# linto-ai/whisper-timestamped

Measured on NVIDIA H100. Metric: audio-sec/s (RTF) large-v3 1h synthetic @1/2/4/8 H100; DTW GB/s vs HBM peak, higher is better.
Workload: dtype bf16x3 tensor-core GEMMs (float32-accurate), f32 elsewhere, f64 DTW accumulate

## Files before the change

### whisper-timestamped_b200/csrc/gemm_tc.cu

```cuda
#include <cuda_bf16.h>

#include <stdlib.h>

#include "sm90.cuh"

namespace wts {

constexpr int BM = 128, BN = 128, BK = 64;
constexpr int TILE_BYTES = BM * BK * 2;
constexpr int STAGES = 3;
constexpr int STAGE_BYTES = 4 * TILE_BYTES;
constexpr int GT_THREADS = 288;
constexpr int PT_THREADS = 384;
constexpr int PT_PRODUCER_REGS = 40, PT_CONSUMER_REGS = 232;
static_assert(128 * PT_PRODUCER_REGS + 256 * PT_CONSUMER_REGS <= 65536, "setmaxnreg plan exceeds the register file");
constexpr int GROUP_M = 8;
constexpr int GT_SMEM = STAGES * STAGE_BYTES + 256 + 1024;
constexpr int PART_LD = BN + 4;
static_assert(BM * PART_LD * 4 <= STAGES * STAGE_BYTES, "the partial tile lives in the operand ring");

__device__ __forceinline__ float gelu_erf_tc(float v) { return 0.5f * v * (1.0f + erff(v * 0.70710678118654752440f)); }

struct TcArgs {
    WtsGemm g;
    int a_has_bo, a_has_bi, b_has_bo, b_has_bi;
    int split_k;
    int pair_stores;
};

__device__ __forceinline__ int64_t out_offset(const WtsGemm& g, int m, int n, int64_t ld)
{
    return g.head_dim > 0 ? (int64_t)(n / g.head_dim) * g.head_stride + (int64_t)m * ld + (n % g.head_dim)
                          : (int64_t)m * ld + n;
}

__device__ __forceinline__ void store_one(const WtsGemm& g, int m, int n, float t, float* of, __nv_bfloat16* ob)
{
    if (of) of[out_offset(g, m, n, g.ldc)] = t;
    if (ob) {
        const __nv_bfloat16 hi = __float2bfloat16_rn(t);
        __nv_bfloat16* d = ob + out_offset(g, m, n, g.ldo);
        d[0] = hi;
        d[g.o_plane] = __float2bfloat16_rn(t - __bfloat162float(hi));
    }
}

__device__ __forceinline__ float2 pair_values(const WtsGemm& g, int n, bool two, float v0, float v1, float bias_m, const float* res)
{
    float t0 = g.alpha * v0, t1 = g.alpha * v1;
    if (g.bias) {
        t0 += g.bias_on_m ? bias_m : g.bias[n];
        if (two) t1 += g.bias_on_m ? bias_m : g.bias[n + 1];
    }
    if (g.act == 1) { t0 = gelu_erf_tc(t0); t1 = gelu_erf_tc(t1); }
    if (res) { t0 += res[n]; if (two) t1 += res[n + 1]; }
    return make_float2(t0, t1);
}

__device__ __forceinline__ void store_pair_sb16(__nv_bfloat16* dh, int64_t plane, float t0, float t1)
{
    const __nv_bfloat162 hi = __floats2bfloat162_rn(t0, t1);
    const __nv_bfloat162 lo = __floats2bfloat162_rn(t0 - __low2float(hi), t1 - __high2float(hi));
    *reinterpret_cast<__nv_bfloat162*>(dh) = hi;
    *reinterpret_cast<__nv_bfloat162*>(dh + plane) = lo;
}

__device__ __forceinline__ void epilogue_pair(const WtsGemm& g, int m, int n, float v0, float v1, float bias_m,
                                              const float* res, float* of, __nv_bfloat16* ob)
{
    const bool two = n + 1 < g.N;
    const float2 t = pair_values(g, n, two, v0, v1, bias_m, res);
    const float t0 = t.x, t1 = t.y;
    const bool same_head = g.head_dim == 0 || (n % g.head_dim) + 1 < g.head_dim;
    if (!(two && same_head)) {
        store_one(g, m, n, t0, of, ob);
        if (two) store_one(g, m, n + 1, t1, of, ob);
        return;
    }
    if (of) {
        float* d = of + out_offset(g, m, n, g.ldc);
        if ((reinterpret_cast<uintptr_t>(d) & 7) == 0) *reinterpret_cast<float2*>(d) = make_float2(t0, t1);
        else { d[0] = t0; d[1] = t1; }
    }
    if (ob) {
        __nv_bfloat16* dh = ob + out_offset(g, m, n, g.ldo);
        __nv_bfloat16* dl = dh + g.o_plane;
        if (((reinterpret_cast<uintptr_t>(dh) | reinterpret_cast<uintptr_t>(dl)) & 3) == 0) {
            store_pair_sb16(dh, g.o_plane, t0, t1);
        } else {
            const __nv_bfloat162 hi = __floats2bfloat162_rn(t0, t1);
            const __nv_bfloat162 lo = __floats2bfloat162_rn(t0 - __low2float(hi), t1 - __high2float(hi));
            dh[0] = hi.x; dh[1] = hi.y; dl[0] = lo.x; dl[1] = lo.y;
        }
    }
}

template <bool PAIRS>
__device__ __forceinline__ void epilogue_frag64(const WtsGemm& g, int zo, int zi, int m_base, int n0, const float (&acc)[64])
{
    const int lane = threadIdx.x & 31;
    const int cl = 2 * (lane & 3);
    float* of = g.out_f32 ? g.out_f32 + (int64_t)zo * g.c_bo + (int64_t)zi * g.c_bi : nullptr;
    __nv_bfloat16* ob = g.out_sb16 ? reinterpret_cast<__nv_bfloat16*>(g.out_sb16) + (int64_t)zo * g.o_bo + (int64_t)zi * g.o_bi : nullptr;
#pragma unroll
    for (int i = 0; i < 2; ++i) {
        const int m = m_base + (lane >> 2) + 8 * i;
        if (m >= g.M || (g.row_mask && g.row_mask[m] == 0)) continue;
        const float* res = g.residual ? g.residual + (int64_t)zo * g.r_bo + (int64_t)zi * g.r_bi + (int64_t)m * g.ldr : nullptr;
        const float bias_m = (g.bias && g.bias_on_m) ? g.bias[m] : 0.f;
#pragma unroll
        for (int j = 0; j < 16; ++j) {
            const int n = n0 + cl + 8 * j;
            if (PAIRS) {
                const float2 t = pair_values(g, n, true, acc[4 * j + 2 * i], acc[4 * j + 2 * i + 1], bias_m, res);
                if (of) *reinterpret_cast<float2*>(of + out_offset(g, m, n, g.ldc)) = t;
                if (ob) store_pair_sb16(ob + out_offset(g, m, n, g.ldo), g.o_plane, t.x, t.y);
            } else if (n < g.N) {
                epilogue_pair(g, m, n, acc[4 * j + 2 * i], acc[4 * j + 2 * i + 1], bias_m, res, of, ob);
            }
        }
    }
}

__device__ __forceinline__ void named_bar_sync(int id, int n) { asm volatile("bar.sync %0, %1;" ::"r"(id), "r"(n) : "memory"); }
__device__ __forceinline__ void named_bar_arrive(int id, int n) { asm volatile("bar.arrive %0, %1;" ::"r"(id), "r"(n) : "memory"); }

struct TileCoord { int m0, n0, zo, zi; };

__device__ __forceinline__ TileCoord tile_coord(const WtsGemm& g, int t, int tiles_m, int tiles_n)
{
    const int per_batch = tiles_m * tiles_n;
    const int z = t / per_batch;
    int r = t - z * per_batch;
    const int span = GROUP_M * tiles_n;
    const int grp = r / span;
    const int m_first = grp * GROUP_M;
    const int gm = min(GROUP_M, tiles_m - m_first);
    r -= grp * span;
    TileCoord c;
    c.m0 = (m_first + r % gm) * BM;
    c.n0 = (r / gm) * BN;
    c.zo = z / g.batch_inner;
    c.zi = z - c.zo * g.batch_inner;
    return c;
}

__global__ void __launch_bounds__(PT_THREADS, 1)
gemm_tc_kernel(const __grid_constant__ CUtensorMap tmA, const __grid_constant__ CUtensorMap tmB, const TcArgs args)
{
    extern __shared__ unsigned char smem_raw[];
    const WtsGemm& g = args.g;
    const uint32_t base = (smem_addr(smem_raw) + 1023u) & ~1023u;
    const uint32_t bar = base + STAGES * STAGE_BYTES;
    const int wg = threadIdx.x >> 7, warp = (threadIdx.x >> 5) & 3, lane = threadIdx.x & 31;
    const int tiles_n = (g.N + BN - 1) / BN, tiles_m = (g.M + BM - 1) / BM;
    const int tiles = tiles_m * tiles_n * g.batch_outer * g.batch_inner;
    const int nkb = (g.K + BK - 1) / BK;
    pdl_launch();

    if (threadIdx.x == 0) {
        asm volatile("prefetch.tensormap [%0];" ::"l"(&tmA) : "memory");
        asm volatile("prefetch.tensormap [%0];" ::"l"(&tmB) : "memory");
        for (int s = 0; s < STAGES; ++s) { mbar_init(bar + 8 * s, 1); mbar_init(bar + 32 + 8 * s, 4); }
        asm volatile("fence.mbarrier_init.release.cluster;" ::: "memory");
    }
    __syncthreads();
    pdl_wait();

    if (wg == 0) {
        asm volatile("setmaxnreg.dec.sync.aligned.u32 %0;" ::"n"(PT_PRODUCER_REGS));
        if (warp == 0 && lane == 0) {
            int p = 0;
            for (int t = blockIdx.x; t < tiles; t += gridDim.x) {
                const TileCoord tc = tile_coord(g, t, tiles_m, tiles_n);
                const int azo = args.a_has_bo ? tc.zo : 0, azi = args.a_has_bi ? tc.zi : 0;
                const int bzo = args.b_has_bo ? tc.zo : 0, bzi = args.b_has_bi ? tc.zi : 0;
                for (int kb = 0; kb < nkb; ++kb, ++p) {
                    const int s = p % STAGES, u = p / STAGES;
                    mbar_wait(bar + 32 + 8 * s, (u & 1) ^ 1);
                    const uint32_t full = bar + 8 * s;
                    mbar_expect_tx(full, STAGE_BYTES);
                    const uint32_t st = base + s * STAGE_BYTES;
                    const int kc = kb * BK;
                    tma_load_5d(st, &tmA, full, kc, tc.m0, azi, azo, 0);
                    tma_load_5d(st + TILE_BYTES, &tmA, full, kc, tc.m0, azi, azo, 1);
                    tma_load_5d(st + 2 * TILE_BYTES, &tmB, full, kc, tc.n0, bzi, bzo, 0);
                    tma_load_5d(st + 3 * TILE_BYTES, &tmB, full, kc, tc.n0, bzi, bzo, 1);
                }
            }
        }
        return;
    }

    asm volatile("setmaxnreg.inc.sync.aligned.u32 %0;" ::"n"(PT_CONSUMER_REGS));
    const int c = wg - 1;
    float acc[2][64];
    int l = c;
    for (int t = blockIdx.x + c * gridDim.x; t < tiles; t += 2 * gridDim.x, l += 2) {
        if (l > 0) named_bar_sync(1 + c, 256);
#pragma unroll
        for (int h = 0; h < 2; ++h)
#pragma unroll
            for (int i = 0; i < 64; ++i) acc[h][i] = 0.f;
        int p = l * nkb;
        for (int kb = 0; kb < nkb; ++kb, ++p) {
            const int s = p % STAGES;
            mbar_wait(bar + 8 * s, (p / STAGES) & 1);
            const uint32_t st = base + s * STAGE_BYTES;
            const uint64_t a_hi = wg_desc(st), a_lo = wg_desc(st + TILE_BYTES);
            const uint64_t b_hi = wg_desc(st + 2 * TILE_BYTES), b_lo = wg_desc(st + 3 * TILE_BYTES);
            constexpr uint64_t a_half = (TILE_BYTES / 2) >> 4;
            wg_fence();
#pragma unroll
            for (int k = 0; k < BK / 16; ++k) {
                const uint64_t adv = (uint64_t)(k * 2);
#pragma unroll
                for (int h = 0; h < 2; ++h) wgmma_ss_n128(acc[h], a_hi + h * a_half + adv, b_hi + adv, 1);
#pragma unroll
                for (int h = 0; h < 2; ++h) wgmma_ss_n128(acc[h], a_lo + h * a_half + adv, b_hi + adv, 1);
#pragma unroll
                for (int h = 0; h < 2; ++h) wgmma_ss_n128(acc[h], a_hi + h * a_half + adv, b_lo + adv, 1);
            }
            wg_commit();
            wg_wait<1>();
            if (kb > 0 && lane == 0) mbar_arrive(bar + 32 + 8 * ((p - 1) % STAGES));
        }
        if (t + gridDim.x < tiles) named_bar_arrive(2 - c, 256);
        wg_wait<0>();
        if (lane == 0) mbar_arrive(bar + 32 + 8 * ((p - 1) % STAGES));

        const TileCoord tc = tile_coord(g, t, tiles_m, tiles_n);
        const bool pairs = args.pair_stores && tc.n0 + BN <= g.N;
#pragma unroll 1
        for (int h = 0; h < 2; ++h) {
            float v[64];
#pragma unroll
            for (int i = 0; i < 64; ++i) v[i] = h ? acc[1][i] : acc[0][i];
            if (pairs) epilogue_frag64<true>(g, tc.zo, tc.zi, tc.m0 + 64 * h + 16 * warp, tc.n0, v);
            else epilogue_frag64<false>(g, tc.zo, tc.zi, tc.m0 + 64 * h + 16 * warp, tc.n0, v);
        }
    }
}

__global__ void __launch_bounds__(GT_THREADS, 1)
gemm_tc_skinny_kernel(const __grid_constant__ CUtensorMap tmA, const __grid_constant__ CUtensorMap tmB, const TcArgs args)
{
    extern __shared__ unsigned char smem_raw[];
    const WtsGemm& g = args.g;
    const uint32_t base = (smem_addr(smem_raw) + 1023u) & ~1023u;
    const uint32_t bar = base + STAGES * STAGE_BYTES;
    const int warp = threadIdx.x >> 5, lane = threadIdx.x & 31;
    const int n0 = blockIdx.x * BN, m0 = blockIdx.y * BM;
    const int S = args.split_k;
    const int z = S > 1 ? 0 : blockIdx.z, zo = z / g.batch_inner, zi = z - zo * g.batch_inner;
    const int nkb_all = (g.K + BK - 1) / BK;
    const int part_k = S > 1 ? blockIdx.z : 0;
    const int kb0 = (int)((int64_t)part_k * nkb_all / S);
    const int nkb = (int)((int64_t)(part_k + 1) * nkb_all / S) - kb0;
    pdl_launch();

    if (threadIdx.x == 256) {
        asm volatile("prefetch.tensormap [%0];" ::"l"(&tmA) : "memory");
        asm volatile("prefetch.tensormap [%0];" ::"l"(&tmB) : "memory");
        for (int s = 0; s < STAGES; ++s) { mbar_init(bar + 8 * s, 1); mbar_init(bar + 32 + 8 * s, 8); }
        asm volatile("fence.mbarrier_init.release.cluster;" ::: "memory");
    }
    __syncthreads();
    pdl_wait();

    float acc[64];
    if (warp == 8) {
        if (lane == 0) {
            const int azo = args.a_has_bo ? zo : 0, azi = args.a_has_bi ? zi : 0;
            const int bzo = args.b_has_bo ? zo : 0, bzi = args.b_has_bi ? zi : 0;
            for (int kb = 0; kb < nkb; ++kb) {
                const int s = kb % STAGES, u = kb / STAGES;
                mbar_wait(bar + 32 + 8 * s, (u & 1) ^ 1);
                const uint32_t full = bar + 8 * s;
                mbar_expect_tx(full, STAGE_BYTES);
                const uint32_t st = base + s * STAGE_BYTES;
                const int kc = (kb0 + kb) * BK;
                tma_load_5d(st, &tmA, full, kc, m0, azi, azo, 0);
                tma_load_5d(st + TILE_BYTES, &tmA, full, kc, m0, azi, azo, 1);
                tma_load_5d(st + 2 * TILE_BYTES, &tmB, full, kc, n0, bzi, bzo, 0);
                tma_load_5d(st + 3 * TILE_BYTES, &tmB, full, kc, n0, bzi, bzo, 1);
            }
        }
    } else {
        const int wg = warp >> 2;
#pragma unroll
        for (int i = 0; i < 64; ++i) acc[i] = 0.f;
        for (int kb = 0; kb < nkb; ++kb) {
            const int s = kb % STAGES, u = kb / STAGES;
            mbar_wait(bar + 8 * s, u & 1);
            const uint32_t st = base + s * STAGE_BYTES;
            const uint64_t a_hi = wg_desc(st + wg * (TILE_BYTES / 2)), a_lo = wg_desc(st + TILE_BYTES + wg * (TILE_BYTES / 2));
            const uint64_t b_hi = wg_desc(st + 2 * TILE_BYTES), b_lo = wg_desc(st + 3 * TILE_BYTES);
            wg_fence();
#pragma unroll
            for (int k = 0; k < BK / 16; ++k) {
                const uint64_t adv = (uint64_t)(k * 2);
                wgmma_ss_n128(acc, a_hi + adv, b_hi + adv, 1);
                wgmma_ss_n128(acc, a_lo + adv, b_hi + adv, 1);
                wgmma_ss_n128(acc, a_hi + adv, b_lo + adv, 1);
            }
            wg_commit();
            wg_wait<1>();
            if (kb > 0 && lane == 0) mbar_arrive(bar + 32 + 8 * ((kb - 1) % STAGES));
        }
        wg_wait<0>();

        const int rl = 64 * wg + 16 * (warp & 3) + (lane >> 2);
        const int cl = 2 * (lane & 3);
        if (S == 1) {
            epilogue_frag64<false>(g, zo, zi, m0 + 64 * wg + 16 * (warp & 3), n0, acc);
        } else {
            asm volatile("bar.sync 1, 256;" ::: "memory");
            float* part = reinterpret_cast<float*>(smem_raw + (base - smem_addr(smem_raw)));
#pragma unroll
            for (int i = 0; i < 2; ++i)
#pragma unroll
                for (int j = 0; j < 16; ++j)
                    *reinterpret_cast<float2*>(part + (rl + 8 * i) * PART_LD + cl + 8 * j) =
                        make_float2(acc[4 * j + 2 * i], acc[4 * j + 2 * i + 1]);
        }
    }
    if (S > 1) {
        __syncwarp();
        cluster_sync_all();
        if (threadIdx.x < 256) {
            uint32_t rank;
            asm volatile("mov.u32 %0, %%cluster_ctarank;" : "=r"(rank));
            const int c = threadIdx.x & 127, half = threadIdx.x >> 7;
            const int n = n0 + c;
            if (n < g.N) {
                uint32_t peer[8];
#pragma unroll
                for (int s = 0; s < 8; ++s) {
                    peer[s] = 0;
                    if (s < S) asm volatile("mapa.shared::cluster.u32 %0, %1, %2;" : "=r"(peer[s]) : "r"(base + 4u * c), "r"(s));
                }
                const float bias_n = (g.bias && !g.bias_on_m) ? g.bias[n] : 0.f;
                float* of = g.out_f32;
                __nv_bfloat16* ob = reinterpret_cast<__nv_bfloat16*>(g.out_sb16);
#pragma unroll 1
                for (int m = (int)rank + S * half; m < g.M; m += 2 * S) {
                    if (g.row_mask && g.row_mask[m] == 0) continue;
                    float x[8];
#pragma unroll
                    for (int s = 0; s < 8; ++s) {
                        x[s] = 0.f;
                        if (s < S) asm volatile("ld.shared::cluster.f32 %0, [%1];" : "=f"(x[s]) : "r"(peer[s] + (uint32_t)(m * PART_LD * 4)));
                    }
                    float t = 0.f;
#pragma unroll
                    for (int s = 0; s < 8; ++s) t += x[s];
                    t = g.alpha * t + (g.bias ? (g.bias_on_m ? g.bias[m] : bias_n) : 0.f);
                    if (g.act == 1) t = gelu_erf_tc(t);
                    if (g.residual) t += g.residual[(int64_t)m * g.ldr + n];
                    store_one(g, m, n, t, of, ob);
                }
            }
        }
        __syncwarp();
        cluster_sync_all();
    }
}

static int make_map(CUtensorMap* tm, const void* ptr, int64_t K, int64_t rows, int64_t ld, int64_t plane, int64_t n_bi,
                    int64_t s_bi, int64_t n_bo, int64_t s_bo, int box_rows, const char* which)
{
    auto enc = tensor_map_encoder();
    if (!enc) { set_error("wts_gemm: cuTensorMapEncodeTiled entry point not available"); return -4; }
    if ((reinterpret_cast<uintptr_t>(ptr) & 15) || (ld & 7) || (plane & 7) || (s_bi & 7) || (s_bo & 7)) {
        set_error("wts_gemm(tc): operand %s not 16-byte aligned (ptr=%p ld=%lld plane=%lld bi=%lld bo=%lld)", which, ptr,
                  (long long)ld, (long long)plane, (long long)s_bi, (long long)s_bo);
        return -5;
    }
    const int64_t e_bi = s_bi ? n_bi : 1, e_bo = s_bo ? n_bo : 1;
    cuuint64_t dims[5] = {(cuuint64_t)K, (cuuint64_t)rows, (cuuint64_t)e_bi, (cuuint64_t)e_bo, 2};
    const cuuint64_t row_b = (cuuint64_t)ld * 2;
    cuuint64_t strides[4] = {row_b, (cuuint64_t)(s_bi ? s_bi * 2 : row_b), (cuuint64_t)(s_bo ? s_bo * 2 : row_b),
                             (cuuint64_t)plane * 2};
    cuuint32_t box[5] = {BK, (cuuint32_t)box_rows, 1, 1, 1};
    cuuint32_t estr[5] = {1, 1, 1, 1, 1};
    CUresult r = enc(tm, CU_TENSOR_MAP_DATA_TYPE_BFLOAT16, 5, const_cast<void*>(ptr), dims, strides, box, estr,
                     CU_TENSOR_MAP_INTERLEAVE_NONE, CU_TENSOR_MAP_SWIZZLE_128B, CU_TENSOR_MAP_L2_PROMOTION_L2_256B,
                     CU_TENSOR_MAP_FLOAT_OOB_FILL_NONE);
    if (r != CUDA_SUCCESS) {
        set_error("wts_gemm(tc): cuTensorMapEncodeTiled(%s) failed with %d (K=%lld rows=%lld ld=%lld plane=%lld)", which, (int)r,
                  (long long)K, (long long)rows, (long long)ld, (long long)plane);
        return -6;
    }
    return 0;
}

int gemm_tc_launch(const WtsGemm& g, cudaStream_t st)
{
    static int n_sm = 0;
    if (n_sm == 0) {
        WTS_CUDA_CHECK(cudaFuncSetAttribute(gemm_tc_kernel, cudaFuncAttributeMaxDynamicSharedMemorySize, GT_SMEM));
        WTS_CUDA_CHECK(cudaFuncSetAttribute(gemm_tc_skinny_kernel, cudaFuncAttributeMaxDynamicSharedMemorySize, GT_SMEM));
        int dev = 0;
        WTS_CUDA_CHECK(cudaGetDevice(&dev));
        WTS_CUDA_CHECK(cudaDeviceGetAttribute(&n_sm, cudaDevAttrMultiProcessorCount, dev));
    }
    alignas(64) CUtensorMap tmA, tmB;
    int rc = make_map(&tmA, g.a, g.K, g.M, g.lda, g.a_plane, g.batch_inner, g.a_bi, g.batch_outer, g.a_bo, BM, "A");
    if (rc) return rc;
    rc = make_map(&tmB, g.b, g.K, g.N, g.ldb, g.b_plane, g.batch_inner, g.b_bi, g.batch_outer, g.b_bo, BN, "B");
    if (rc) return rc;
    TcArgs args;
    args.g = g;
    args.a_has_bo = g.a_bo != 0; args.a_has_bi = g.a_bi != 0;
    args.b_has_bo = g.b_bo != 0; args.b_has_bi = g.b_bi != 0;
    const int tiles_n = (g.N + BN - 1) / BN, tiles_m = (g.M + BM - 1) / BM, nkb = (g.K + BK - 1) / BK;
    const int batch = g.batch_outer * g.batch_inner;
    cudaLaunchConfig_t cfg = {};
    cfg.dynamicSmemBytes = GT_SMEM;
    cfg.stream = st;
    const bool skinny = tiles_m == 1 && batch == 1 && g.head_dim == 0;
    if (!skinny) {
        const int64_t tiles = (int64_t)tiles_m * tiles_n * batch;
        if (tiles > INT32_MAX / 2) { set_error("wts_gemm(tc): %lld output tiles are too many", (long long)tiles); return -7; }
        args.split_k = 1;
        const bool heads_even = g.head_dim == 0 || (g.head_dim % 2 == 0 && g.head_stride % 2 == 0);
        const bool of_pairs = !g.out_f32 || ((reinterpret_cast<uintptr_t>(g.out_f32) & 7) == 0 && g.ldc % 2 == 0 &&
                                             g.c_bo % 2 == 0 && g.c_bi % 2 == 0);
        const bool ob_pairs = !g.out_sb16 || ((reinterpret_cast<uintptr_t>(g.out_sb16) & 3) == 0 && g.ldo % 2 == 0 &&
                                              g.o_plane % 2 == 0 && g.o_bo % 2 == 0 && g.o_bi % 2 == 0);
        args.pair_stores = !g.row_mask && heads_even && of_pairs && ob_pairs;
        cfg.gridDim = dim3((unsigned)(tiles < n_sm ? tiles : n_sm), 1, 1);
        cfg.blockDim = dim3(PT_THREADS, 1, 1);
        WTS_CUDA_CHECK(cudaLaunchKernelEx(&cfg, gemm_tc_kernel, tmA, tmB, args));
        return 0;
    }
    static const int splitk = []{ const char* e = getenv("WTS_SPLITK"); return e ? atoi(e) : 1; }();
    int split = 1;
    if (splitk && 2 * tiles_n <= n_sm) {
        split = n_sm / tiles_n;
        if (split > 8) split = 8;
        if (split > nkb) split = nkb;
    }
    args.split_k = split;
    args.pair_stores = 0;
    cfg.gridDim = dim3(tiles_n, 1, split);
    cfg.blockDim = dim3(GT_THREADS, 1, 1);
    cudaLaunchAttribute attr[2];
    int na = 0;
    if (split > 1) {
        attr[na].id = cudaLaunchAttributeClusterDimension;
        attr[na].val.clusterDim.x = 1;
        attr[na].val.clusterDim.y = 1;
        attr[na].val.clusterDim.z = split;
        ++na;
    }
    if (pdl_enabled()) {
        attr[na].id = cudaLaunchAttributeProgrammaticStreamSerialization;
        attr[na].val.programmaticStreamSerializationAllowed = 1;
        ++na;
    }
    cfg.attrs = attr;
    cfg.numAttrs = na;
    WTS_CUDA_CHECK(cudaLaunchKernelEx(&cfg, gemm_tc_skinny_kernel, tmA, tmB, args));
    return 0;
}

}
```

### whisper-timestamped_b200/csrc/ops.cu

```cuda
#include "decode_common.cuh"

namespace wts {

__global__ void to_sb16_kernel(const float* __restrict__ x, int64_t n, __nv_bfloat16* __restrict__ hi,
                               __nv_bfloat16* __restrict__ lo)
{
    for (int64_t i = blockIdx.x * (int64_t)blockDim.x + threadIdx.x; i < n; i += (int64_t)gridDim.x * blockDim.x) {
        __nv_bfloat16 h, l;
        split_bf16(x[i], h, l);
        hi[i] = h;
        lo[i] = l;
    }
}

constexpr int LN_THREADS = 128, LN_MAXV = 16;
__global__ void __launch_bounds__(LN_THREADS)
layernorm_kernel(const float* x, int64_t ldx, const float* gamma,
                 const float* beta, int M, int D, __nv_bfloat16* o, int64_t ldo,
                 int64_t o_plane, float* of, int64_t ldf)
{
    pdl_launch();
    pdl_wait();
    __shared__ float red[32];
    const int row = blockIdx.x;
    const float* xr = x + (int64_t)row * ldx;
    float v[LN_MAXV];
    float s = 0.f;
#pragma unroll
    for (int k = 0; k < LN_MAXV; ++k) {
        const int c = threadIdx.x + LN_THREADS * k;
        v[k] = c < D ? xr[c] : 0.f;
        s += v[k];
    }
    const float mean = block_reduce_sum(s, red) / (float)D;
    float q = 0.f;
#pragma unroll
    for (int k = 0; k < LN_MAXV; ++k) {
        const int c = threadIdx.x + LN_THREADS * k;
        const float d = c < D ? v[k] - mean : 0.f;
        q += d * d;
    }
    const float rstd = 1.0f / sqrtf(block_reduce_sum(q, red) / (float)D + 1e-5f);
#pragma unroll
    for (int k = 0; k < LN_MAXV; ++k) {
        const int c = threadIdx.x + LN_THREADS * k;
        if (c < D) {
            const float y = (v[k] - mean) * rstd * gamma[c] + beta[c];
            if (o) {
                __nv_bfloat16 h, l;
                split_bf16(y, h, l);
                o[(int64_t)row * ldo + c] = h;
                o[(int64_t)row * ldo + c + o_plane] = l;
            }
            if (of) of[(int64_t)row * ldf + c] = y;
        }
    }
}

__global__ void __launch_bounds__(128)
softmax_rows_kernel(const float* __restrict__ s, int64_t lds, int64_t rows, int n,
                    __nv_bfloat16* __restrict__ o, int64_t ldo, int64_t o_plane)
{
    const int64_t row = (int64_t)blockIdx.x * 4 + (threadIdx.x >> 5);
    const int lane = threadIdx.x & 31;
    if (row >= rows) return;
    const float* sr = s + row * lds;
    float v[64];
    float mx = -CUDART_INF_F;
#pragma unroll
    for (int k = 0; k < 64; ++k) {
        const int c = lane + 32 * k;
        v[k] = c < n ? sr[c] : -CUDART_INF_F;
        mx = fmaxf(mx, v[k]);
    }
    mx = warp_max(mx);
    float sum = 0.f;
#pragma unroll
    for (int k = 0; k < 64; ++k) {
        v[k] = expf(v[k] - mx);
        sum += v[k];
    }
    sum = warp_sum(sum);
    const float inv = 1.0f / sum;
#pragma unroll
    for (int k = 0; k < 64; ++k) {
        const int c = lane + 32 * k;
        if (c < n) {
            __nv_bfloat16 h, l;
            split_bf16(v[k] * inv, h, l);
            o[row * ldo + c] = h;
            o[row * ldo + c + o_plane] = l;
        }
    }
}

__global__ void frames_kernel(const float* __restrict__ audio, int64_t n_samples, int64_t n_total,
                              int64_t n_frames, float* __restrict__ out)
{
    const int64_t t = blockIdx.x;
    if (t >= n_frames) return;
    for (int n = threadIdx.x; n < 400; n += blockDim.x) {
        int64_t i = t * 160 - 200 + n;
        if (i < 0) i = -i;
        if (i >= n_total) i = 2 * (n_total - 1) - i;
        const float x = (i >= 0 && i < n_samples) ? audio[i] : 0.f;
        const float w = 0.5f - 0.5f * cospif((float)n / 200.0f);
        out[t * 400 + n] = x * w;
    }
}

__global__ void power_kernel(const float* __restrict__ y, int64_t ldy, int64_t n_frames, float* __restrict__ p,
                             int64_t ldp)
{
    const int64_t i = blockIdx.x * (int64_t)blockDim.x + threadIdx.x;
    if (i >= n_frames * 208) return;
    const int64_t t = i / 208;
    const int k = (int)(i - t * 208);
    const float re = y[t * ldy + k], im = y[t * ldy + 208 + k];
    p[t * ldp + k] = re * re + im * im;
}

__device__ __forceinline__ float mel_log10(float m) { return log10f(fmaxf(m, 1e-10f)); }

__global__ void logmel_max_kernel(const float* __restrict__ m, int64_t n, float* __restrict__ out)
{
    __shared__ float red[32];
    float mx = -CUDART_INF_F;
    for (int64_t i = blockIdx.x * (int64_t)blockDim.x + threadIdx.x; i < n; i += (int64_t)gridDim.x * blockDim.x)
        mx = fmaxf(mx, mel_log10(m[i]));
    mx = block_reduce_max(mx, red);
    if (threadIdx.x == 0) {
        int key = __float_as_int(mx);
        key = key >= 0 ? key : key ^ 0x7fffffff;
        atomicMax(reinterpret_cast<int*>(out), key);
    }
}

__global__ void logmel_finish_kernel(const float* __restrict__ m, int64_t n, const float* __restrict__ mxkey,
                                     float* __restrict__ out)
{
    int key = *reinterpret_cast<const int*>(mxkey);
    key = key >= 0 ? key : key ^ 0x7fffffff;
    const float gmax = __int_as_float(key);
    for (int64_t i = blockIdx.x * (int64_t)blockDim.x + threadIdx.x; i < n; i += (int64_t)gridDim.x * blockDim.x) {
        float x = mel_log10(m[i]);
        x = fmaxf(x, gmax - 8.0f);
        out[i] = (x + 4.0f) / 4.0f;
    }
}

__global__ void window_gather_kernel(const int64_t* __restrict__ mel_ptr, int n_mels,
                                     const int32_t* __restrict__ seek, const int32_t* __restrict__ size, int B,
                                     __nv_bfloat16* __restrict__ out, int64_t o_plane)
{
    const int b = blockIdx.y;
    const float* mel = reinterpret_cast<const float*>(mel_ptr[b]);
    const int64_t i = blockIdx.x * (int64_t)blockDim.x + threadIdx.x;
    const int64_t per = (int64_t)3002 * n_mels;
    if (i >= per) return;
    const int r = (int)(i / n_mels), c = (int)(i - (int64_t)r * n_mels);
    float v = 0.f;
    const int t = r - 1;
    if (t >= 0 && t < size[b]) v = mel[((int64_t)seek[b] + t) * n_mels + c];
    __nv_bfloat16 h, l;
    split_bf16(v, h, l);
    out[b * per + i] = h;
    out[b * per + i + o_plane] = l;
}

__global__ void embed_kernel(const int32_t* tokens, const int32_t* positions,
                             const float* emb, const float* pos, int rows, int D,
                             float* out)
{
    pdl_launch();
    pdl_wait();
    const int r = blockIdx.x;
    if (r >= rows) return;
    const float* e = emb + (int64_t)tokens[r] * D;
    const float* p = pos + (int64_t)positions[r] * D;
    for (int c = threadIdx.x; c < D; c += blockDim.x) out[(int64_t)r * D + c] = e[c] + p[c];
}

__global__ void gather_rows_kernel(const float* __restrict__ x, int64_t ldx, const int32_t* __restrict__ idx,
                                   int rows, int D, float* __restrict__ out)
{
    const int r = blockIdx.x;
    if (r >= rows) return;
    const float* s = x + (int64_t)idx[r] * ldx;
    for (int c = threadIdx.x; c < D; c += blockDim.x) out[(int64_t)r * D + c] = s[c];
}

constexpr int DA_THREADS = 128;
__global__ void __launch_bounds__(DA_THREADS)
decoder_attention_kernel(const int kind, const float* q, int64_t ldq, const float* kc,
                         const float* vc, int64_t seq_stride, int ctx,
                         const int32_t* row_seq, const int32_t* row_pos, int H,
                         __nv_bfloat16* o, int64_t ldo, int64_t o_plane, float* qk_out,
                         const int32_t* head_slot, int n_slots, int qk_rows,
                         const int32_t* qk_row, const int32_t* row_active)
{
    pdl_launch();
    pdl_wait();
    extern __shared__ float sm[];
    float* sc = sm;
    float* qs = sm + ctx;
    float* red = qs + 64;
    float* part = red + 32;
    const int r = blockIdx.x, h = blockIdx.y;
    if (row_active != nullptr && !row_active[r]) return;
    const int seq = row_seq[r];
    const int nk = kind == 1 ? ctx : row_pos[r] + 1;
    const float* K = kc + (int64_t)seq * seq_stride + (int64_t)h * ctx * 64;
    const float* V = vc + (int64_t)seq * seq_stride + (int64_t)h * ctx * 64;
    if (kind == 2) {
        const float* src = q + (int64_t)r * ldq + h * 64;
        const int64_t at = (int64_t)(nk - 1) * 64 + (threadIdx.x & 63);
        if (threadIdx.x < 64) const_cast<float*>(K)[at] = src[(int64_t)H * 64 + threadIdx.x];
        else                  const_cast<float*>(V)[at] = src[(int64_t)2 * H * 64 + (threadIdx.x & 63)];
    }
    if (threadIdx.x < 64) qs[threadIdx.x] = q[(int64_t)r * ldq + h * 64 + threadIdx.x];
    __syncthreads();
    float mx = -CUDART_INF_F;
    for (int j = threadIdx.x; j < nk; j += DA_THREADS) {
        const float4* kr = reinterpret_cast<const float4*>(K + (int64_t)j * 64);
        float acc = 0.f;
#pragma unroll
        for (int c = 0; c < 16; ++c) {
            const float4 kv = kr[c];
            acc += qs[4 * c] * kv.x + qs[4 * c + 1] * kv.y + qs[4 * c + 2] * kv.z + qs[4 * c + 3] * kv.w;
        }
        sc[j] = acc;
        mx = fmaxf(mx, acc);
    }
    __syncthreads();
    if (kind == 1 && qk_out != nullptr) {
        const int slot = head_slot[h];
        const int qr = qk_row[r];
        if (slot >= 0 && qr >= 0) {
            float* dst = qk_out + (((int64_t)seq * n_slots + slot) * qk_rows + qr) * (int64_t)ctx;
            for (int j = threadIdx.x; j < nk; j += DA_THREADS) dst[j] = sc[j];
        }
    }
    mx = block_reduce_max(mx, red);
    float sum = 0.f;
    for (int j = threadIdx.x; j < nk; j += DA_THREADS) {
        const float e = expf(sc[j] - mx);
        sc[j] = e;
        sum += e;
    }
    sum = block_reduce_sum(sum, red);
    const float inv = 1.0f / sum;
    const int c = threadIdx.x & 63, g = threadIdx.x >> 6;
    float acc = 0.f;
    for (int j = g; j < nk; j += 2) acc += sc[j] * V[(int64_t)j * 64 + c];
    part[g * 64 + c] = acc;
    __syncthreads();
    if (threadIdx.x < 64) {
        const float y = (part[threadIdx.x] + part[64 + threadIdx.x]) * inv;
        __nv_bfloat16 hi, lo;
        split_bf16(y, hi, lo);
        o[(int64_t)r * ldo + h * 64 + threadIdx.x] = hi;
        o[(int64_t)r * ldo + h * 64 + threadIdx.x + o_plane] = lo;
    }
}


__global__ void cross_kv_pack_kernel(const float* __restrict__ src, __half* __restrict__ dst16,
                                     float* __restrict__ dst_align, const int32_t* __restrict__ head_slot,
                                     int s0, int n_l, int H, int ctx)
{
    const int bh = blockIdx.x;
    const int b = bh / H, h = bh - b * H;
    const float* s = src + (int64_t)bh * ctx * 64;
    __half* d = dst16 + (int64_t)bh * ctx * 64;
    const int slot = dst_align ? head_slot[h] : -1;
    float* da = slot >= 0 ? dst_align + ((int64_t)b * n_l + slot - s0) * ctx * 64 : nullptr;
    for (int i = threadIdx.x; i < ctx * 64; i += blockDim.x) {
        const float v = s[i];
        d[i] = __float2half_rn(v);
        if (da) da[i] = v;
    }
}

__global__ void __launch_bounds__(CA_THREADS)
cross_attention_f16_kernel(const float* q, int64_t ldq, const __half* k16,
                           const __half* v16, const float* k_align,
                           const int32_t* head_slot, int n_slots, int s0, int n_l, int ctx,
                           const int32_t* row_seq, int H, __nv_bfloat16* o, int64_t ldo,
                           int64_t o_plane, float* qk_out, int qk_rows, const int32_t* qk_row,
                           const int32_t* row_active)
{
    pdl_launch();
    pdl_wait();
    __shared__ CaScratch sc;
    const int r = blockIdx.x, h = blockIdx.y;
    if (row_active != nullptr && !row_active[r]) return;
    const int seq = row_seq[r];
    const int slot = head_slot[h];
    const int c8 = threadIdx.x & 7;
    float qf[8];
    {
        const float4* qp = reinterpret_cast<const float4*>(q + (int64_t)r * ldq + h * 64 + c8 * 8);
        const float4 a = qp[0], b = qp[1];
        qf[0] = a.x; qf[1] = a.y; qf[2] = a.z; qf[3] = a.w; qf[4] = b.x; qf[5] = b.y; qf[6] = b.z; qf[7] = b.w;
    }
    const __half* V = v16 + ((int64_t)seq * H + h) * ctx * 64;
    float* qk_dst = nullptr;
    const float* kal = nullptr;
    if (slot >= 0) {
        kal = k_align + ((int64_t)seq * n_l + slot - s0) * ctx * 64;
        if (qk_out != nullptr) {
            const int qr = qk_row[r];
            if (qr >= 0) qk_dst = qk_out + (((int64_t)seq * n_slots + slot) * qk_rows + qr) * (int64_t)ctx;
        }
    }
    const float y = ca_row_head<4>(qf, k16 + ((int64_t)seq * H + h) * ctx * 64, V, kal, qk_dst, ctx, sc);
    if (threadIdx.x < 64) {
        __nv_bfloat16 hi, lo;
        split_bf16(y, hi, lo);
        o[(int64_t)r * ldo + h * 64 + threadIdx.x] = hi;
        o[(int64_t)r * ldo + h * 64 + threadIdx.x + o_plane] = lo;
    }
}

__global__ void kv_append_kernel(const float* k, const float* v, int64_t ld,
                                 const int32_t* row_seq, const int32_t* row_pos, int H,
                                 int ctx, float* kc, float* vc, int64_t seq_stride)
{
    pdl_launch();
    pdl_wait();
    const int r = blockIdx.x;
    const int seq = row_seq[r], pos = row_pos[r];
    for (int c = threadIdx.x; c < H * 64; c += blockDim.x) {
        const int h = c >> 6, d = c & 63;
        const int64_t dst = (int64_t)seq * seq_stride + ((int64_t)h * ctx + pos) * 64 + d;
        kc[dst] = k[(int64_t)r * ld + c];
        vc[dst] = v[(int64_t)r * ld + c];
    }
}

constexpr int DS_THREADS = 1024;
__global__ void __launch_bounds__(DS_THREADS)
decode_select_kernel(float* logits, int64_t ldl, const WtsDecodeCfg cfg,
                     const uint8_t* suppress, const uint8_t* blank,
                     int32_t* tokens, int32_t* n_tokens,
                     const int32_t* n_prompt, int32_t* done,
                     float* logprobs, int lp_ld, float* full, float* last_full)
{
    pdl_launch();
    pdl_wait();
    __shared__ SelectScratch S;
    const int b = blockIdx.x;
    if (done[b]) return;
    select_row(logits + (int64_t)b * ldl, cfg, suppress, blank, tokens + (int64_t)b * cfg.tokens_ld, n_tokens + b,
               n_prompt[b], done + b, logprobs + (int64_t)b * lp_ld,
               full != nullptr ? full + (int64_t)b * lp_ld * cfg.n_vocab : nullptr,
               last_full != nullptr ? last_full + (int64_t)b * cfg.n_vocab : nullptr, S);
}

__global__ void __launch_bounds__(DS_THREADS)
filtered_logprobs_kernel(const float* logits, int64_t ldl, const WtsDecodeCfg cfg, const uint8_t* suppress, const uint8_t* blank,
                         int32_t* tokens, int32_t* n_tokens, const int32_t* n_prompt, float* out)
{
    __shared__ SelectScratch S;
    const int b = blockIdx.x;
    select_row(logits + (int64_t)b * ldl, cfg, suppress, blank, tokens + (int64_t)b * cfg.tokens_ld, n_tokens + b,
               n_prompt[b], nullptr, nullptr, out + (int64_t)b * cfg.n_vocab, nullptr, S, true);
}

__global__ void step_inputs_kernel(const int32_t* tokens, int ld, const int32_t* n_tokens,
                                   const int32_t* n_prompt, const int32_t* done, int B,
                                   int32_t* tok, int32_t* pos, int32_t* qk_row,
                                   int32_t* active)
{
    pdl_launch();
    pdl_wait();
    const int b = blockIdx.x * blockDim.x + threadIdx.x;
    if (b >= B) return;
    const int nt = n_tokens[b];
    tok[b] = tokens[(int64_t)b * ld + nt - 1];
    pos[b] = nt - 1;
    qk_row[b] = done[b] ? -1 : nt - n_prompt[b];
    if (active) active[b] = done[b] ? 0 : 1;
}

__global__ void softmax_pick_kernel(const float* __restrict__ logits, int64_t ldl, int n, int index,
                                    float* __restrict__ out)
{
    __shared__ float red[32];
    const float* x = logits + (int64_t)blockIdx.x * ldl;
    float mx = -CUDART_INF_F;
    for (int v = threadIdx.x; v < n; v += blockDim.x) mx = fmaxf(mx, x[v]);
    mx = block_reduce_max(mx, red);
    float s = 0.f;
    for (int v = threadIdx.x; v < n; v += blockDim.x) s += expf(x[v] - mx);
    s = block_reduce_sum(s, red);
    if (threadIdx.x == 0) out[blockIdx.x] = expf(x[index] - mx) / s;
}

__global__ void logprob_gather_kernel(const float* logits, int64_t ldl, int n, const int32_t* rows, const int32_t* tokens,
                                      float* out)
{
    __shared__ float red[32];
    const float* x = logits + (int64_t)rows[blockIdx.x] * ldl;
    float mx = -CUDART_INF_F;
    for (int v = threadIdx.x; v < n; v += blockDim.x) mx = fmaxf(mx, x[v]);
    mx = block_reduce_max(mx, red);
    float s = 0.f;
    for (int v = threadIdx.x; v < n; v += blockDim.x) s += expf(x[v] - mx);
    s = block_reduce_sum(s, red);
    if (threadIdx.x == 0) out[blockIdx.x] = (x[tokens[blockIdx.x]] - mx) - logf(s);
}

}

using namespace wts;

static inline int grid_for(int64_t n, int block, int cap = 132 * 16)
{
    int64_t g = (n + block - 1) / block;
    return (int)(g < 1 ? 1 : (g > cap ? cap : g));
}

extern "C" int wts_to_sb16(const float* d_x, int64_t n, void* d_hi, void* d_lo, void* stream)
{
    if (n <= 0) return 0;
    to_sb16_kernel<<<grid_for(n, 256), 256, 0, (cudaStream_t)stream>>>(d_x, n, (__nv_bfloat16*)d_hi, (__nv_bfloat16*)d_lo);
    WTS_LAUNCH_CHECK();
    return 0;
}

extern "C" int wts_layernorm(const float* d_x, int64_t ldx, const float* d_gamma, const float* d_beta, int32_t M,
                             int32_t D, void* d_out_sb16, int64_t ldo, int64_t o_plane, float* d_out_f32,
                             int64_t ldf, void* stream)
{
    if (M <= 0) return 0;
    if (D > LN_THREADS * LN_MAXV) { set_error("wts_layernorm: D=%d > %d", D, LN_THREADS * LN_MAXV); return -2; }
    WTS_CUDA_CHECK(launch_pdl(layernorm_kernel, dim3(M), dim3(LN_THREADS), 0, (cudaStream_t)stream, d_x, ldx, d_gamma, d_beta, M, D,
                                                                   (__nv_bfloat16*)d_out_sb16, ldo, o_plane, d_out_f32, ldf));
    WTS_LAUNCH_CHECK();
    return 0;
}

extern "C" int wts_softmax_rows(const float* d_s, int64_t lds, int64_t rows, int32_t n, void* d_out_sb16,
                                int64_t ldo, int64_t o_plane, void* stream)
{
    if (rows <= 0) return 0;
    if (n > 2048) { set_error("wts_softmax_rows: n=%d > 2048", n); return -2; }
    softmax_rows_kernel<<<(unsigned)((rows + 3) / 4), 128, 0, (cudaStream_t)stream>>>(d_s, lds, rows, n,
                                                                                     (__nv_bfloat16*)d_out_sb16, ldo, o_plane);
    WTS_LAUNCH_CHECK();
    return 0;
}

extern "C" int wts_frames(const float* d_audio, int64_t n_samples, int64_t n_total, int64_t n_frames, void* d_out,
                          int64_t o_plane, void* stream)
{
    (void)o_plane;
    if (n_frames <= 0) return 0;
    frames_kernel<<<(unsigned)n_frames, 128, 0, (cudaStream_t)stream>>>(d_audio, n_samples, n_total, n_frames, (float*)d_out);
    WTS_LAUNCH_CHECK();
    return 0;
}

extern "C" int wts_power(const float* d_y, int64_t ldy, int64_t n_frames, void* d_out, int64_t ldo, int64_t o_plane,
                         void* stream)
{
    (void)o_plane;
    if (n_frames <= 0) return 0;
    power_kernel<<<(unsigned)((n_frames * 208 + 255) / 256), 256, 0, (cudaStream_t)stream>>>(d_y, ldy, n_frames, (float*)d_out, ldo);
    WTS_LAUNCH_CHECK();
    return 0;
}

extern "C" int wts_logmel_max(const float* d_m, int64_t n, float* d_max, void* stream)
{
    logmel_max_kernel<<<grid_for(n, 256, 1024), 256, 0, (cudaStream_t)stream>>>(d_m, n, d_max);
    WTS_LAUNCH_CHECK();
    return 0;
}

extern "C" int wts_logmel_finish(const float* d_m, int64_t n_frames, int32_t n_mels, const float* d_max,
                                 float* d_out_f32, void* stream)
{
    const int64_t n = n_frames * n_mels;
    logmel_finish_kernel<<<grid_for(n, 256), 256, 0, (cudaStream_t)stream>>>(d_m, n, d_max, d_out_f32);
    WTS_LAUNCH_CHECK();
    return 0;
}

extern "C" int wts_window_gather(const int64_t* d_mel_ptr, int32_t n_mels, const int32_t* d_seek,
                                 const int32_t* d_size, int32_t B, void* d_out, int64_t o_plane, void* stream)
{
    if (B <= 0) return 0;
    dim3 grid((unsigned)(((int64_t)3002 * n_mels + 255) / 256), B);
    window_gather_kernel<<<grid, 256, 0, (cudaStream_t)stream>>>(d_mel_ptr, n_mels, d_seek, d_size, B,
                                                                 (__nv_bfloat16*)d_out, o_plane);
    WTS_LAUNCH_CHECK();
    return 0;
}

extern "C" int wts_embed(const int32_t* d_tokens, const int32_t* d_positions, const float* d_emb, const float* d_pos,
                         int32_t rows, int32_t D, float* d_out, void* stream)
{
    if (rows <= 0) return 0;
    WTS_CUDA_CHECK(launch_pdl(embed_kernel, dim3(rows), dim3(256), 0, (cudaStream_t)stream, d_tokens, d_positions, d_emb, d_pos, rows, D, d_out));
    WTS_LAUNCH_CHECK();
    return 0;
}

extern "C" int wts_gather_rows(const float* d_x, int64_t ldx, const int32_t* d_idx, int32_t rows, int32_t D,
                               float* d_out, void* stream)
{
    if (rows <= 0) return 0;
    gather_rows_kernel<<<rows, 256, 0, (cudaStream_t)stream>>>(d_x, ldx, d_idx, rows, D, d_out);
    WTS_LAUNCH_CHECK();
    return 0;
}

extern "C" int wts_decoder_attention(int32_t kind, const float* d_q, int64_t ldq, const float* d_k, const float* d_v,
                                     int64_t seq_stride, int32_t ctx, const int32_t* d_row_seq,
                                     const int32_t* d_row_pos, int32_t rows, int32_t H, void* d_out_sb16, int64_t ldo,
                                     int64_t o_plane, float* d_qk_out, const int32_t* d_head_slot, int32_t n_slots,
                                     int32_t qk_rows, const int32_t* d_qk_row, const int32_t* d_row_active, void* stream)
{
    if (rows <= 0) return 0;
    const size_t smem = ((size_t)ctx + 64 + 32 + 128) * sizeof(float);
    dim3 grid(rows, H);
    WTS_CUDA_CHECK(launch_pdl(decoder_attention_kernel, grid, dim3(DA_THREADS), smem, (cudaStream_t)stream, 
        kind, d_q, ldq, d_k, d_v, seq_stride, ctx, d_row_seq, d_row_pos, H, (__nv_bfloat16*)d_out_sb16, ldo, o_plane,
        d_qk_out, d_head_slot, n_slots, qk_rows, d_qk_row, d_row_active));
    WTS_LAUNCH_CHECK();
    return 0;
}


extern "C" int wts_cross_kv_pack_layer(const float* d_src, void* d_dst16, float* d_dst_align,
                                       const int32_t* d_head_slot, int32_t align_s0, int32_t align_n, int32_t B,
                                       int32_t H, int32_t ctx, void* stream)
{
    if (B <= 0) return 0;
    cross_kv_pack_kernel<<<B * H, 256, 0, (cudaStream_t)stream>>>(d_src, (__half*)d_dst16, d_dst_align, d_head_slot,
                                                                 align_s0, align_n, H, ctx);
    WTS_LAUNCH_CHECK();
    return 0;
}

extern "C" int wts_cross_kv_pack(const float* d_src, void* d_dst16, float* d_dst_align, const int32_t* d_head_slot,
                                 int32_t n_slots, int32_t B, int32_t H, int32_t ctx, void* stream)
{
    return wts_cross_kv_pack_layer(d_src, d_dst16, d_dst_align, d_head_slot, 0, n_slots, B, H, ctx, stream);
}

extern "C" int wts_cross_attention_f16_layer(const float* d_q, int64_t ldq, const void* d_k16, const void* d_v16,
                                             const float* d_k_align, const int32_t* d_head_slot, int32_t n_slots,
                                             int32_t align_s0, int32_t align_n, int32_t ctx, const int32_t* d_row_seq,
                                             int32_t rows, int32_t H, void* d_out_sb16, int64_t ldo, int64_t o_plane,
                                             float* d_qk_out, int32_t qk_rows, const int32_t* d_qk_row,
                                             const int32_t* d_row_active, void* stream)
{
    if (rows <= 0) return 0;
    if ((ldq & 3) || (reinterpret_cast<uintptr_t>(d_q) & 15)) { set_error("wts_cross_attention_f16: q must be 16-byte aligned"); return -2; }
    dim3 grid(rows, H);
    WTS_CUDA_CHECK(launch_pdl(cross_attention_f16_kernel, grid, dim3(CA_THREADS), 0, (cudaStream_t)stream, 
        d_q, ldq, (const __half*)d_k16, (const __half*)d_v16, d_k_align, d_head_slot, n_slots, align_s0, align_n, ctx,
        d_row_seq, H, (__nv_bfloat16*)d_out_sb16, ldo, o_plane, d_qk_out, qk_rows, d_qk_row, d_row_active));
    WTS_LAUNCH_CHECK();
    return 0;
}

extern "C" int wts_cross_attention_f16(const float* d_q, int64_t ldq, const void* d_k16, const void* d_v16,
                                       const float* d_k_align, const int32_t* d_head_slot, int32_t n_slots,
                                       int32_t ctx, const int32_t* d_row_seq, int32_t rows, int32_t H,
                                       void* d_out_sb16, int64_t ldo, int64_t o_plane, float* d_qk_out,
                                       int32_t qk_rows, const int32_t* d_qk_row, const int32_t* d_row_active,
                                       void* stream)
{
    return wts_cross_attention_f16_layer(d_q, ldq, d_k16, d_v16, d_k_align, d_head_slot, n_slots, 0, n_slots, ctx,
                                         d_row_seq, rows, H, d_out_sb16, ldo, o_plane, d_qk_out, qk_rows, d_qk_row,
                                         d_row_active, stream);
}

extern "C" int wts_kv_append(const float* d_k, const float* d_v, int64_t ld, const int32_t* d_row_seq,
                             const int32_t* d_row_pos, int32_t rows, int32_t H, int32_t ctx, float* d_kc, float* d_vc,
                             int64_t seq_stride, void* stream)
{
    if (rows <= 0) return 0;
    WTS_CUDA_CHECK(launch_pdl(kv_append_kernel, dim3(rows), dim3(256), 0, (cudaStream_t)stream, d_k, d_v, ld, d_row_seq, d_row_pos, H, ctx, d_kc, d_vc, seq_stride));
    WTS_LAUNCH_CHECK();
    return 0;
}

extern "C" int wts_decode_select(float* d_logits, int64_t ldl, const WtsDecodeCfg* cfg, const uint8_t* d_suppress,
                                 const uint8_t* d_blank, int32_t* d_tokens, int32_t* d_n_tokens,
                                 const int32_t* d_n_prompt, int32_t* d_done, float* d_logprobs, int32_t lp_ld,
                                 float* d_full_logprobs, float* d_last_full, int32_t B, void* stream)
{
    if (B <= 0) return 0;
    WTS_CUDA_CHECK(launch_pdl(decode_select_kernel, dim3(B), dim3(DS_THREADS), 0, (cudaStream_t)stream, d_logits, ldl, *cfg, d_suppress, d_blank, d_tokens,
                                                                    d_n_tokens, d_n_prompt, d_done, d_logprobs, lp_ld,
                                                                    d_full_logprobs, d_last_full));
    WTS_LAUNCH_CHECK();
    return 0;
}

extern "C" int wts_filtered_logprobs(const float* d_logits, int64_t ldl, const WtsDecodeCfg* cfg, const uint8_t* d_suppress,
                                     const uint8_t* d_blank, int32_t* d_tokens, int32_t* d_n_tokens, const int32_t* d_n_prompt,
                                     float* d_out, int32_t B, void* stream)
{
    if (B <= 0) return 0;
    if (!d_logits || !cfg || !d_suppress || !d_blank || !d_tokens || !d_n_tokens || !d_n_prompt || !d_out) {
        set_error("wts_filtered_logprobs: null pointer");
        return -2;
    }
    filtered_logprobs_kernel<<<B, DS_THREADS, 0, (cudaStream_t)stream>>>(d_logits, ldl, *cfg, d_suppress, d_blank, d_tokens,
                                                                         d_n_tokens, d_n_prompt, d_out);
    WTS_LAUNCH_CHECK();
    return 0;
}

extern "C" int wts_step_inputs(const int32_t* d_tokens, int32_t tokens_ld, const int32_t* d_n_tokens,
                               const int32_t* d_n_prompt, const int32_t* d_done, int32_t B, int32_t* d_tok,
                               int32_t* d_pos, int32_t* d_qk_row, int32_t* d_active, void* stream)
{
    if (B <= 0) return 0;
    WTS_CUDA_CHECK(launch_pdl(step_inputs_kernel, dim3((B + 127) / 128), dim3(128), 0, (cudaStream_t)stream, d_tokens, tokens_ld, d_n_tokens, d_n_prompt,
                                                                         d_done, B, d_tok, d_pos, d_qk_row, d_active));
    WTS_LAUNCH_CHECK();
    return 0;
}

extern "C" int wts_softmax_pick(const float* d_logits, int64_t ldl, int32_t n, int32_t index, float* d_out,
                                int32_t rows, void* stream)
{
    if (rows <= 0) return 0;
    softmax_pick_kernel<<<rows, 512, 0, (cudaStream_t)stream>>>(d_logits, ldl, n, index, d_out);
    WTS_LAUNCH_CHECK();
    return 0;
}

extern "C" int wts_logprob_gather(const float* d_logits, int64_t ldl, int32_t n, const int32_t* d_rows,
                                  const int32_t* d_tokens, float* d_out, int32_t count, void* stream)
{
    if (count <= 0) return 0;
    if (!d_logits || !d_rows || !d_tokens || !d_out) { set_error("wts_logprob_gather: null pointer"); return -2; }
    logprob_gather_kernel<<<count, 512, 0, (cudaStream_t)stream>>>(d_logits, ldl, n, d_rows, d_tokens, d_out);
    WTS_LAUNCH_CHECK();
    return 0;
}
```

Measured before the change: 611.3.

## Add a 64-row decode GEMM kernel with two CTAs per SM

Adds a specialised tensor-core GEMM for skinny decode shapes (M<=64). It uses a single consumer warpgroup, a 64-row A tile, and two pipeline stages, so two CTAs fit on one SM and more weight streams run concurrently. The split-K cluster reduction is factored into a shared helper. Separately, the decoder self-attention and cross-attention launches drop programmatic dependent launch in favour of plain launches. That removes PDL overlap for those kernels, possibly because of a correctness concern.

After: 633.7 (median of 6 runs). 3.7% higher.

```diff
diff --git a/whisper-timestamped_b200/csrc/gemm_tc.cu b/whisper-timestamped_b200/csrc/gemm_tc.cu
--- a/whisper-timestamped_b200/csrc/gemm_tc.cu
+++ b/whisper-timestamped_b200/csrc/gemm_tc.cu
@@ -18,6 +18,14 @@
 constexpr int GT_SMEM = STAGES * STAGE_BYTES + 256 + 1024;
 constexpr int PART_LD = BN + 4;
 static_assert(BM * PART_LD * 4 <= STAGES * STAGE_BYTES, "the partial tile lives in the operand ring");
+constexpr int DM = 64;
+constexpr int DA_BYTES = DM * BK * 2;
+constexpr int DSTAGES = 2;
+constexpr int DSTAGE_BYTES = 2 * DA_BYTES + 2 * TILE_BYTES;
+constexpr int DT_THREADS = 160;
+constexpr int DT_SMEM = DSTAGES * DSTAGE_BYTES + 256 + 1024;
+static_assert(DM * PART_LD * 4 <= DSTAGES * DSTAGE_BYTES, "the partial tile lives in the operand ring");
+static_assert(2 * (DT_SMEM + 1024) <= 228 * 1024, "two decode CTAs share an SM");
 
 __device__ __forceinline__ float gelu_erf_tc(float v) { return 0.5f * v * (1.0f + erff(v * 0.70710678118654752440f)); }
 
@@ -242,6 +250,38 @@
     }
 }
 
+__device__ __forceinline__ void splitk_reduce(const WtsGemm& g, uint32_t base, int n0, int S, int c, int m_begin, int m_step)
+{
+    const int n = n0 + c;
+    if (n >= g.N) return;
+    uint32_t peer[8];
+#pragma unroll
+    for (int s = 0; s < 8; ++s) {
+        peer[s] = 0;
+        if (s < S) asm volatile("mapa.shared::cluster.u32 %0, %1, %2;" : "=r"(peer[s]) : "r"(base + 4u * c), "r"(s));
+    }
+    const float bias_n = (g.bias && !g.bias_on_m) ? g.bias[n] : 0.f;
+    float* of = g.out_f32;
+    __nv_bfloat16* ob = reinterpret_cast<__nv_bfloat16*>(g.out_sb16);
+#pragma unroll 1
+    for (int m = m_begin; m < g.M; m += m_step) {
+        if (g.row_mask && g.row_mask[m] == 0) continue;
+        float x[8];
+#pragma unroll
+        for (int s = 0; s < 8; ++s) {
+            x[s] = 0.f;
+            if (s < S) asm volatile("ld.shared::cluster.f32 %0, [%1];" : "=f"(x[s]) : "r"(peer[s] + (uint32_t)(m * PART_LD * 4)));
+        }
+        float t = 0.f;
+#pragma unroll
+        for (int s = 0; s < 8; ++s) t += x[s];
+        t = g.alpha * t + (g.bias ? (g.bias_on_m ? g.bias[m] : bias_n) : 0.f);
+        if (g.act == 1) t = gelu_erf_tc(t);
+        if (g.residual) t += g.residual[(int64_t)m * g.ldr + n];
+        store_one(g, m, n, t, of, ob);
+    }
+}
+
 __global__ void __launch_bounds__(GT_THREADS, 1)
 gemm_tc_skinny_kernel(const __grid_constant__ CUtensorMap tmA, const __grid_constant__ CUtensorMap tmB, const TcArgs args)
 {
@@ -331,36 +371,104 @@
         if (threadIdx.x < 256) {
             uint32_t rank;
             asm volatile("mov.u32 %0, %%cluster_ctarank;" : "=r"(rank));
-            const int c = threadIdx.x & 127, half = threadIdx.x >> 7;
-            const int n = n0 + c;
-            if (n < g.N) {
-                uint32_t peer[8];
-#pragma unroll
-                for (int s = 0; s < 8; ++s) {
-                    peer[s] = 0;
-                    if (s < S) asm volatile("mapa.shared::cluster.u32 %0, %1, %2;" : "=r"(peer[s]) : "r"(base + 4u * c), "r"(s));
+            splitk_reduce(g, base, n0, S, threadIdx.x & 127, (int)rank + S * (threadIdx.x >> 7), 2 * S);
+        }
+        __syncwarp();
+        cluster_sync_all();
+    }
+}
+
+__global__ void __launch_bounds__(DT_THREADS, 2)
+gemm_tc_decode_kernel(const __grid_constant__ CUtensorMap tmA, const __grid_constant__ CUtensorMap tmB, const TcArgs args)
+{
+    extern __shared__ unsigned char smem_raw[];
+    const WtsGemm& g = args.g;
+    const uint32_t base = (smem_addr(smem_raw) + 1023u) & ~1023u;
+    const uint32_t bar = base + DSTAGES * DSTAGE_BYTES;
+    const int warp = threadIdx.x >> 5, lane = threadIdx.x & 31;
+    const int n0 = blockIdx.x * BN;
+    const int S = args.split_k;
+    const int nkb_all = (g.K + BK - 1) / BK;
+    const int kb0 = (int)((int64_t)blockIdx.z * nkb_all / S);
+    const int nkb = (int)((int64_t)(blockIdx.z + 1) * nkb_all / S) - kb0;
+    pdl_launch();
+
+    if (threadIdx.x == 128) {
+        asm volatile("prefetch.tensormap [%0];" ::"l"(&tmA) : "memory");
+        asm volatile("prefetch.tensormap [%0];" ::"l"(&tmB) : "memory");
+        for (int s = 0; s < DSTAGES; ++s) { mbar_init(bar + 8 * s, 1); mbar_init(bar + 32 + 8 * s, 4); }
+        asm volatile("fence.mbarrier_init.release.cluster;" ::: "memory");
+        for (int kb = 0; kb < DSTAGES && kb < nkb; ++kb) {
+            const uint32_t st = base + kb * DSTAGE_BYTES, full = bar + 8 * kb;
+            mbar_expect_tx(full, DSTAGE_BYTES);
+            tma_load_5d(st + 2 * DA_BYTES, &tmB, full, (kb0 + kb) * BK, n0, 0, 0, 0);
+            tma_load_5d(st + 2 * DA_BYTES + TILE_BYTES, &tmB, full, (kb0 + kb) * BK, n0, 0, 0, 1);
+        }
+    }
+    __syncthreads();
+    pdl_wait();
+
+    if (warp == 4) {
+        if (lane == 0) {
+            for (int kb = 0; kb < nkb; ++kb) {
+                const int s = kb % DSTAGES, u = kb / DSTAGES;
+                const uint32_t full = bar + 8 * s, st = base + s * DSTAGE_BYTES;
+                const int kc = (kb0 + kb) * BK;
+                if (kb >= DSTAGES) {
+                    mbar_wait(bar + 32 + 8 * s, (u & 1) ^ 1);
+                    mbar_expect_tx(full, DSTAGE_BYTES);
+                    tma_load_5d(st + 2 * DA_BYTES, &tmB, full, kc, n0, 0, 0, 0);
+                    tma_load_5d(st + 2 * DA_BYTES + TILE_BYTES, &tmB, full, kc, n0, 0, 0, 1);
                 }
-                const float bias_n = (g.bias && !g.bias_on_m) ? g.bias[n] : 0.f;
-                float* of = g.out_f32;
-                __nv_bfloat16* ob = reinterpret_cast<__nv_bfloat16*>(g.out_sb16);
-#pragma unroll 1
-                for (int m = (int)rank + S * half; m < g.M; m += 2 * S) {
-                    if (g.row_mask && g.row_mask[m] == 0) continue;
-                    float x[8];
-#pragma unroll
-                    for (int s = 0; s < 8; ++s) {
-                        x[s] = 0.f;
-                        if (s < S) asm volatile("ld.shared::cluster.f32 %0, [%1];" : "=f"(x[s]) : "r"(peer[s] + (uint32_t)(m * PART_LD * 4)));
-                    }
-                    float t = 0.f;
-#pragma unroll
-                    for (int s = 0; s < 8; ++s) t += x[s];
-                    t = g.alpha * t + (g.bias ? (g.bias_on_m ? g.bias[m] : bias_n) : 0.f);
-                    if (g.act == 1) t = gelu_erf_tc(t);
-                    if (g.residual) t += g.residual[(int64_t)m * g.ldr + n];
-                    store_one(g, m, n, t, of, ob);
-                }
-            }
+                tma_load_5d(st, &tmA, full, kc, 0, 0, 0, 0);
+                tma_load_5d(st + DA_BYTES, &tmA, full, kc, 0, 0, 0, 1);
+            }
+        }
+    } else {
+        float acc[64];
+#pragma unroll
+        for (int i = 0; i < 64; ++i) acc[i] = 0.f;
+        for (int kb = 0; kb < nkb; ++kb) {
+            const int s = kb % DSTAGES, u = kb / DSTAGES;
+            mbar_wait(bar + 8 * s, u & 1);
+            const uint32_t st = base + s * DSTAGE_BYTES;
+            const uint64_t a_hi = wg_desc(st), a_lo = wg_desc(st + DA_BYTES);
+            const uint64_t b_hi = wg_desc(st + 2 * DA_BYTES), b_lo = wg_desc(st + 2 * DA_BYTES + TILE_BYTES);
+            wg_fence();
+#pragma unroll
+            for (int k = 0; k < BK / 16; ++k) {
+                const uint64_t adv = (uint64_t)(k * 2);
+                wgmma_ss_n128(acc, a_hi + adv, b_hi + adv, 1);
+                wgmma_ss_n128(acc, a_lo + adv, b_hi + adv, 1);
+                wgmma_ss_n128(acc, a_hi + adv, b_lo + adv, 1);
+            }
+            wg_commit();
+            wg_wait<1>();
+            if (kb > 0 && lane == 0) mbar_arrive(bar + 32 + 8 * ((kb - 1) % DSTAGES));
+        }
+        wg_wait<0>();
+
+        if (S == 1) {
+            epilogue_frag64<false>(g, 0, 0, 16 * warp, n0, acc);
+        } else {
+            asm volatile("bar.sync 1, 128;" ::: "memory");
+            const int rl = 16 * warp + (lane >> 2), cl = 2 * (lane & 3);
+            float* part = reinterpret_cast<float*>(smem_raw + (base - smem_addr(smem_raw)));
+#pragma unroll
+            for (int i = 0; i < 2; ++i)
+#pragma unroll
+                for (int j = 0; j < 16; ++j)
+                    *reinterpret_cast<float2*>(part + (rl + 8 * i) * PART_LD + cl + 8 * j) =
+                        make_float2(acc[4 * j + 2 * i], acc[4 * j + 2 * i + 1]);
+        }
+    }
+    if (S > 1) {
+        __syncwarp();
+        cluster_sync_all();
+        if (threadIdx.x < 128) {
+            uint32_t rank;
+            asm volatile("mov.u32 %0, %%cluster_ctarank;" : "=r"(rank));
+            splitk_reduce(g, base, n0, S, threadIdx.x, (int)rank, S);
         }
         __syncwarp();
         cluster_sync_all();
@@ -401,6 +509,9 @@
     if (n_sm == 0) {
         WTS_CUDA_CHECK(cudaFuncSetAttribute(gemm_tc_kernel, cudaFuncAttributeMaxDynamicSharedMemorySize, GT_SMEM));
         WTS_CUDA_CHECK(cudaFuncSetAttribute(gemm_tc_skinny_kernel, cudaFuncAttributeMaxDynamicSharedMemorySize, GT_SMEM));
+        WTS_CUDA_CHECK(cudaFuncSetAttribute(gemm_tc_decode_kernel, cudaFuncAttributeMaxDynamicSharedMemorySize, DT_SMEM));
+        WTS_CUDA_CHECK(cudaFuncSetAttribute(gemm_tc_decode_kernel, cudaFuncAttributePreferredSharedMemoryCarveout,
+                                            cudaSharedmemCarveoutMaxShared));
         int dev = 0;
         WTS_CUDA_CHECK(cudaGetDevice(&dev));
         WTS_CUDA_CHECK(cudaDeviceGetAttribute(&n_sm, cudaDevAttrMultiProcessorCount, dev));
@@ -444,8 +555,14 @@
     }
     args.split_k = split;
     args.pair_stores = 0;
+    const bool decode = g.M <= DM;
+    if (decode) {
+        rc = make_map(&tmA, g.a, g.K, g.M, g.lda, g.a_plane, 1, 0, 1, 0, DM, "A");
+        if (rc) return rc;
+        cfg.dynamicSmemBytes = DT_SMEM;
+    }
     cfg.gridDim = dim3(tiles_n, 1, split);
-    cfg.blockDim = dim3(GT_THREADS, 1, 1);
+    cfg.blockDim = dim3(decode ? DT_THREADS : GT_THREADS, 1, 1);
     cudaLaunchAttribute attr[2];
     int na = 0;
     if (split > 1) {
@@ -462,7 +579,7 @@
     }
     cfg.attrs = attr;
     cfg.numAttrs = na;
-    WTS_CUDA_CHECK(cudaLaunchKernelEx(&cfg, gemm_tc_skinny_kernel, tmA, tmB, args));
+    WTS_CUDA_CHECK(cudaLaunchKernelEx(&cfg, decode ? gemm_tc_decode_kernel : gemm_tc_skinny_kernel, tmA, tmB, args));
     return 0;
 }
 
diff --git a/whisper-timestamped_b200/csrc/ops.cu b/whisper-timestamped_b200/csrc/ops.cu
--- a/whisper-timestamped_b200/csrc/ops.cu
+++ b/whisper-timestamped_b200/csrc/ops.cu
@@ -527,9 +527,9 @@
     if (rows <= 0) return 0;
     const size_t smem = ((size_t)ctx + 64 + 32 + 128) * sizeof(float);
     dim3 grid(rows, H);
-    WTS_CUDA_CHECK(launch_pdl(decoder_attention_kernel, grid, dim3(DA_THREADS), smem, (cudaStream_t)stream, 
+    decoder_attention_kernel<<<grid, DA_THREADS, smem, (cudaStream_t)stream>>>(
         kind, d_q, ldq, d_k, d_v, seq_stride, ctx, d_row_seq, d_row_pos, H, (__nv_bfloat16*)d_out_sb16, ldo, o_plane,
-        d_qk_out, d_head_slot, n_slots, qk_rows, d_qk_row, d_row_active));
+        d_qk_out, d_head_slot, n_slots, qk_rows, d_qk_row, d_row_active);
     WTS_LAUNCH_CHECK();
     return 0;
 }
@@ -562,9 +562,9 @@
     if (rows <= 0) return 0;
     if ((ldq & 3) || (reinterpret_cast<uintptr_t>(d_q) & 15)) { set_error("wts_cross_attention_f16: q must be 16-byte aligned"); return -2; }
     dim3 grid(rows, H);
-    WTS_CUDA_CHECK(launch_pdl(cross_attention_f16_kernel, grid, dim3(CA_THREADS), 0, (cudaStream_t)stream, 
+    cross_attention_f16_kernel<<<grid, CA_THREADS, 0, (cudaStream_t)stream>>>(
         d_q, ldq, (const __half*)d_k16, (const __half*)d_v16, d_k_align, d_head_slot, n_slots, align_s0, align_n, ctx,
-        d_row_seq, H, (__nv_bfloat16*)d_out_sb16, ldo, o_plane, d_qk_out, qk_rows, d_qk_row, d_row_active));
+        d_row_seq, H, (__nv_bfloat16*)d_out_sb16, ldo, o_plane, d_qk_out, qk_rows, d_qk_row, d_row_active);
     WTS_LAUNCH_CHECK();
     return 0;
 }
```
